# wenet-e2e/wenet

Hardware: AMD Instinct MI355X
Metric: audio-seconds/sec (RTF^-1), 12L Conformer fbank80, ctc_prefix_beam_search (higher is better)
Workload: dtype f32 (feed-forward and subsampling-conv2 GEMMs: fp32 operands as three exact bf16 planes, six plane products on the bf16 matrix cores, f32 accumulate -- error <= the v_mfma_f32 kernel's, tests/test_gpu_x6.py; everything else v_mfma_f32)

## Files before the change

### include/wenet_amd.h

```cpp
#ifndef WENET_AMD_H_
#define WENET_AMD_H_

#include <stdint.h>

#ifdef __cplusplus
extern "C" {
#endif

typedef struct wn_model wn_model;

typedef struct {
  int32_t feat_dim;
  int32_t d_model;
  int32_t n_heads;
  int32_t ffn_dim;
  int32_t n_layers;
  int32_t cnn_kernel;
  int32_t causal;
  int32_t use_dynamic_chunk;
  int32_t static_chunk_size;
  int32_t vocab;
  int32_t has_cmvn;
  int32_t dec_heads;
  int32_t dec_ffn_dim;
// ... 179 lines not shown
                    const float* resid_dev, float* C_dev, int32_t M, int32_t N,
                    int32_t K, float alpha, int32_t act, void* stream);
int wn_op_gemm_skinny(const float* A_dev, const float* W_dev, const float* bias_dev,
                      const float* resid_dev, float* C_dev, int32_t M, int32_t N, int32_t K,
                      int32_t act, int32_t w_bf16, int32_t split_k, void* stream);
int wn_op_gemm_bf16_stored(const float* A_dev, const float* W_dev, const float* bias_dev,
                           const float* resid_dev, void* C_dev, int32_t M, int32_t N,
                           int32_t K, float alpha, int32_t act, int32_t c_bf16,
                           void* stream);
int wn_op_gemm_lowp(const void* A_dev, const void* W_dev, const void* a_scale_dev,
                    const void* w_scale_dev, const float* bias_dev,
                    const float* resid_dev, void* C_dev, void* c_scale_dev, int32_t M,
                    int32_t N, int32_t K, float alpha, int32_t act, int32_t c_mode,
                    int32_t dtype, void* stream);
int wn_op_mx_quantize(const float* x_dev, int32_t rows, int32_t K, void* q_dev,
                      void* scale_dev, void* stream);
int wn_op_ffn_fused(const float* X_dev, const float* W1_dev, const float* b1_dev,
                    const float* W2_dev, const float* b2_dev, float* x_inout_dev,
                    const float* ln_w_dev, const float* ln_b_dev, float* y_out_dev,
                    int32_t M, int32_t D, int32_t F, int32_t act, float alpha, float eps,
                    void* stream);
int wn_op_gemm_x6(const float* A_dev, const float* W_dev, const float* bias_dev,
                  const float* resid_dev, float* C_dev, int32_t M, int32_t N, int32_t K,
                  float alpha, int32_t act, int32_t bm, int32_t reps, void* stream);
int wn_op_ffn_x6(const float* X_dev, const float* W1_dev, const float* b1_dev,
                 const float* W2_dev, const float* b2_dev, float* x_inout_dev,
                 const float* ln_w_dev, const float* ln_b_dev, float* y_out_dev, int32_t M,
                 int32_t D, int32_t F, int32_t act, float alpha, float eps, int32_t reps,
                 void* stream);
int wn_op_gemm_x6r(const float* A_dev, const float* W_dev, const float* bias_dev,
                   float* x_inout_dev, const float* ln_w_dev, const float* ln_b_dev,
                   float* y_dev, float* C_dev, int32_t M, int32_t N, int32_t epi, float alpha,
                   float eps, int32_t reps, void* stream);

int wn_op_gemm_x6r512(const float* A, const float* W, const float* bias, float* x_inout,
                      const float* ln_w, const float* ln_b, float* y, const float* W2,
                      const float* bias2, float* C, int32_t M, int32_t N, int32_t epi, float alpha,
                      float eps, int32_t reps, void* stream);
int wn_op_log_add(const double* a_dev, const double* b_dev, double* out_dev,
                  int32_t n, void* stream);
int wn_op_layernorm(const float* x_dev, const float* w_dev, const float* b_dev,
                    float* y_dev, int32_t M, int32_t D, float eps, void* stream);

typedef struct wn_attention_op {
  const void* Q; const void* K; const void* V;
  int32_t ldq, ldk, ldv;
  int32_t q_rows, kv_rows;
  const float* P; int32_t ldp, p_rows;
  const int32_t* p_off;
  const float* bias_u; const float* bias_v;
  void* O; int32_t ldo;
  const int32_t* q_off; const int32_t* q_len;
  const int32_t* kv_off; const int32_t* kv_len;
  int32_t n_seq, n_heads;
  int32_t mask_mode, chunk_size, left_chunks;
  float scale;
  int32_t flags;
  int32_t precision;
  int32_t x6_galign;
} wn_attention_op;
#define WN_ATTN_FOLD 1
#define WN_ATTN_PREFOLD 2
#define WN_ATTN_QKV_BF16 4
#define WN_ATTN_O_BF16 8
int wn_op_attention(const wn_attention_op* op, int32_t* form_out, void* stream);
int wn_op_dwconv(const float* x, int32_t ldx, const float* wt, const float* bias,
// ... 59 lines not shown
```

### wenet_amd/_lib.py

```python
import ctypes
import os
from ctypes import (POINTER, Structure, c_char_p, c_double, c_float, c_int32,
                    c_int64, c_void_p)

_HERE = os.path.dirname(os.path.abspath(__file__))
LIB_PATH = os.path.join(_HERE, 'libwenet_amd.so')


class WnConfig(Structure):
    _fields_ = [(n, c_int32) for n in (
        'feat_dim', 'd_model', 'n_heads', 'ffn_dim', 'n_layers', 'cnn_kernel',
        'causal', 'use_dynamic_chunk', 'static_chunk_size', 'vocab',
        'has_cmvn', 'dec_heads', 'dec_ffn_dim', 'dec_layers', 'dec_r_layers',
        'bidirectional', 'sos', 'eos', 'max_pos')] + [('norm_eps', c_float)] + [
            (n, c_int32) for n in ('encoder_type', 'input_layer', 'activation',
                                   'key_bias', 'cnn_norm',
                                   'dec_activation', 'dec_key_bias', 'dec_src_key_bias',
                                   'dec_learned_pos', 'dec_max_pos')]


class WnTransducerConfig(Structure):
    _fields_ = [(n, c_int32) for n in ('pred_embed', 'pred_hidden', 'pred_layers', 'pred_out',
                                       'join_dim', 'blank')]


class WnTensor(Structure):
    _fields_ = [('name', c_char_p), ('data', POINTER(c_float)),
                ('numel', c_int64)]


class WnStreamResult(Structure):
    _fields_ = [('n_hyps', POINTER(c_int32)), ('hyp_lens', POINTER(c_int32)),
                ('hyp_tlens', POINTER(c_int32)), ('hyp_tokens', POINTER(c_int32)),
                ('hyp_times', POINTER(c_int32)), ('hyp_scores', POINTER(c_double)),
                ('hyp_viterbi', POINTER(c_double)), ('frames_decoded', POINTER(c_int32)),
                ('trailing_blank', POINTER(c_int32)), ('max_len', c_int32)]


class WnAttentionOp(Structure):
    _fields_ = [('Q', c_void_p), ('K', c_void_p), ('V', c_void_p),
                ('ldq', c_int32), ('ldk', c_int32), ('ldv', c_int32),
                ('q_rows', c_int32), ('kv_rows', c_int32),
                ('P', c_void_p), ('ldp', c_int32), ('p_rows', c_int32),
                ('p_off', POINTER(c_int32)), ('bias_u', c_void_p), ('bias_v', c_void_p),
                ('O', c_void_p), ('ldo', c_int32),
                ('q_off', POINTER(c_int32)), ('q_len', POINTER(c_int32)),
                ('kv_off', POINTER(c_int32)), ('kv_len', POINTER(c_int32)),
                ('n_seq', c_int32), ('n_heads', c_int32), ('mask_mode', c_int32),
                ('chunk_size', c_int32), ('left_chunks', c_int32), ('scale', c_float),
                ('flags', c_int32), ('precision', c_int32), ('x6_galign', c_int32)]


EXPORTS = [
    'wn_last_error', 'wn_version', 'wn_model_create', 'wn_model_destroy', 'wn_model_clone',
    'wn_model_set_precision', 'wn_model_get_precision', 'wn_batch_size', 'wn_model_set_encode_gate', 'wn_op_gemm_bf16',
    'wn_op_gemm_bf16_stored',
    'wn_attention_beam_search', 'wn_attention_beam_search_prompt', 'wn_attention_truncated',
    'wn_op_gemm_skinny', 'wn_encode_chunk_batch', 'wn_op_gemm_lowp', 'wn_op_mx_quantize', 'wn_op_ffn_fused', 'wn_op_gemm_x6', 'wn_op_ffn_x6', 'wn_op_gemm_x6r', 'wn_op_gemm_x6r512', 'wn_profile_kernel_name', 'wn_profile_ffn_split', 'wn_profile_ffn_clocks', 'wn_profile_gemm_clocks', 'wn_filter_blank_embedding',
    'wn_workspace_create', 'wn_resample_length', 'wn_resample', 'wn_fbank', 'wn_log_mel', 'wn_encode', 'wn_encode_chunk', 'wn_set_encoder_out',
    'wn_ctc_logprobs', 'wn_set_ctc_probs', 'wn_ctc_greedy_search', 'wn_ctc_force_align',
    'wn_set_context_graph', 'wn_ctc_prefix_beam_search', 'wn_attention_rescoring', 'wn_rescore', 'wn_rescore_prefetch', 'wn_decoder_forward', 'wn_decoder_next_topk', 'wn_op_gemm',
    'wn_op_layernorm', 'wn_op_log_add', 'wn_op_attention', 'wn_op_dwconv', 'wn_op_conv1',
    'wn_op_ctc_rows', 'wn_debug_set', 'wn_profile_enable',
    'wn_profile_collect', 'wn_tune_set', 'wn_model_tune_set', 'wn_tune_get',
    'wn_stream_create', 'wn_stream_destroy', 'wn_stream_set_endpoint', 'wn_stream_reset',
    'wn_stream_advance', 'wn_stream_advance_encoded',
    'wn_model_create_transducer', 'wn_transducer_greedy_search', 'wn_op_lstm_step',
    'wn_op_joint_argmax',
]

_lib = None


def lib():
    global _lib
    if _lib is not None:
        return _lib
    if not os.path.exists(LIB_PATH):
        raise RuntimeError(
            f'{LIB_PATH} is missing: build it with `python -m wenet_amd.build` '
            '(hipcc --offload-arch=gfx950). wenet_amd has no CPU fallback.')
    import torch
    L = ctypes.CDLL(LIB_PATH, mode=ctypes.RTLD_GLOBAL)
    i32, i64, f32, vp = c_int32, c_int64, c_float, c_void_p
    pi32, pf64 = POINTER(c_int32), POINTER(c_double)
    L.wn_last_error.restype = c_char_p
    L.wn_profile_kernel_name.restype = c_char_p
    L.wn_profile_kernel_name.argtypes = [vp]
    L.wn_profile_ffn_split.restype = c_int32
    L.wn_profile_ffn_split.argtypes = [vp]
    L.wn_profile_ffn_clocks.argtypes = [POINTER(ctypes.c_uint64)]
# ... 29 lines not shown
    L.wn_stream_create.argtypes = [vp, i32, i32, i32, i32, POINTER(vp), vp]
    L.wn_stream_destroy.argtypes = [vp]
    L.wn_stream_set_endpoint.argtypes = [vp, f32, f32]
    L.wn_stream_reset.argtypes = [vp, i32, pi32, vp]
    L.wn_stream_advance.argtypes = [vp, i32, pi32, vp, pi32, i32, i32, i32,
                                    POINTER(WnStreamResult), vp]
    L.wn_stream_advance_encoded.argtypes = [vp, i32, pi32, vp, pi32, i32, i32,
                                            POINTER(WnStreamResult), vp]
    L.wn_attention_rescoring.argtypes = [vp, i32, pi32, pi32, pi32, i32, f32,
                                         POINTER(f32), POINTER(f32), vp]
    L.wn_rescore.argtypes = [vp, i32, pi32, pi32, pi32, pf64, i32, c_double, c_double, pi32,
                             POINTER(f32), pf64, pf64, POINTER(f32), vp]
    L.wn_rescore_prefetch.argtypes = [vp, i32, vp]
    L.wn_decoder_forward.argtypes = [vp, i32, i32, i32, pi32, pi32, i32, vp, vp]
    L.wn_decoder_next_topk.argtypes = [vp, i32, pi32, pi32, pi32, i32, i32,
                                       POINTER(f32), pi32, vp]
    L.wn_attention_beam_search.argtypes = [vp, i32, i32, f32, pi32, pi32, vp]
    L.wn_attention_beam_search_prompt.argtypes = [vp, i32, i32, f32, pi32, i32, pi32, pi32, vp]
    L.wn_attention_truncated.argtypes = [vp]
    L.wn_op_gemm.argtypes = [vp, vp, vp, vp, vp, i32, i32, i32, f32, i32, vp]
    L.wn_op_gemm_skinny.argtypes = [vp, vp, vp, vp, vp, i32, i32, i32, i32, i32, i32, vp]
    L.wn_op_gemm_bf16.argtypes = L.wn_op_gemm.argtypes
    L.wn_op_gemm_bf16_stored.argtypes = [vp, vp, vp, vp, vp, i32, i32, i32, f32, i32, i32, vp]
    L.wn_op_gemm_lowp.argtypes = [vp, vp, vp, vp, vp, vp, vp, vp, i32, i32, i32, f32, i32, i32,
                                  i32, vp]
    L.wn_op_mx_quantize.argtypes = [vp, i32, i32, vp, vp, vp]
    L.wn_op_ffn_fused.argtypes = [vp, vp, vp, vp, vp, vp, vp, vp, vp, i32, i32, i32, i32, f32,
                                  f32, vp]
    L.wn_op_gemm_x6.argtypes = [vp, vp, vp, vp, vp, i32, i32, i32, f32, i32, i32, i32, vp]
    L.wn_op_ffn_x6.argtypes = [vp, vp, vp, vp, vp, vp, vp, vp, vp, i32, i32, i32, i32, f32,
                               f32, i32, vp]
    L.wn_filter_blank_embedding.argtypes = [vp, vp, pi32, pi32, vp]
    L.wn_op_gemm_x6r.argtypes = [vp, vp, vp, vp, vp, vp, vp, vp, i32, i32, i32, f32, f32, i32, vp]
    L.wn_op_gemm_x6r512.argtypes = [vp, vp, vp, vp, vp, vp, vp, vp, vp, vp, i32, i32, i32, f32, f32,
                                    i32, vp]
    L.wn_model_set_precision.argtypes = [vp, i32]
    L.wn_model_get_precision.argtypes = [vp]
    L.wn_batch_size.argtypes = [vp]
    L.wn_batch_size.restype = i32
    L.wn_model_set_encode_gate.argtypes = [vp, vp]
    L.wn_op_layernorm.argtypes = [vp, vp, vp, vp, i32, i32, f32, vp]
    L.wn_op_log_add.argtypes = [vp, vp, vp, i32, vp]
    L.wn_op_attention.argtypes = [POINTER(WnAttentionOp), pi32, vp]
    L.wn_op_dwconv.argtypes = [vp, i32, vp, vp, vp, vp, vp, i32, vp, i32, pi32, pi32, i32, i32,
                               i32, i32, i32, i32, f32, vp]
    L.wn_op_conv1.argtypes = [vp, vp, vp, vp, vp, vp, pi32, pi32, i32, i32, i32, i32, i32, i32,
                              vp]
    L.wn_op_ctc_rows.argtypes = [vp, i32, i32, i32, i32, i32, f32, vp, vp, vp, i32, vp]
    L.wn_debug_set.argtypes = [vp, c_char_p, i32]
    L.wn_tune_set.argtypes = [c_char_p, i32]
    L.wn_model_tune_set.argtypes = [vp, c_char_p, i32]
    L.wn_tune_get.argtypes = [vp, c_char_p, pi32]
    L.wn_profile_enable.argtypes = [vp, i32]
    L.wn_profile_collect.argtypes = [vp, pi32, pf64, pf64]
    L.wn_model_create_transducer.argtypes = [POINTER(WnConfig), POINTER(WnTransducerConfig),
                                             POINTER(WnTensor), i32, i32, POINTER(vp)]
    L.wn_transducer_greedy_search.argtypes = [vp, i32, pi32, pi32, i32, pi32, vp]
    L.wn_op_lstm_step.argtypes = [vp, POINTER(vp), i32, vp, vp, vp, vp, vp, vp, i32, i32, i32,
                                  i32, vp]
    L.wn_op_joint_argmax.argtypes = [vp, i32, vp, i32, pi32, pi32, vp, vp, i32, i32, i32, pi32,
                                     POINTER(f32), vp]
    for n in EXPORTS:
        if n not in ('wn_last_error', 'wn_version', 'wn_model_destroy',
                     'wn_resample_length', 'wn_profile_kernel_name',
                     'wn_profile_ffn_split'):
            getattr(L, n).restype = i32
# ... 29 lines not shown
```

### wenet_amd/csrc/cabi_ops.hip

```cpp
#include "model_state.h"
#include "x6.h"

namespace wn {
namespace {

__global__ __launch_bounds__(256) void conv1_image_unpack_kernel(
    const char* __restrict__ img, int tiles, const int* __restrict__ t1_off,
    const int* __restrict__ t1_len, int F1, int C, float* __restrict__ out) {
  const int b = blockIdx.y;
  const int n = t1_len[b] * F1 * (C / 8);
  const int ne = (F1 + 1) / 2;
  for (int i = blockIdx.x * 256 + threadIdx.x; i < n; i += gridDim.x * 256) {
    const int cg = i % (C / 8), px = i / (C / 8);
    const int fr = px / F1, pos = px - fr * F1;
    const int f1 = pos < ne ? 2 * pos : 2 * (pos - ne) + 1;
    const int row = (t1_off[b] + fr) * F1;
    const char* src = img + x3_piece(cg >> 1, tiles, row + pos, cg & 1);
    const bf16x8 p0 = *reinterpret_cast<const bf16x8*>(src);
    const bf16x8 p1 = *reinterpret_cast<const bf16x8*>(src + X3_REC);
    const bf16x8 p2 = *reinterpret_cast<const bf16x8*>(src + 2 * X3_REC);
    float* o = out + ((int64_t)row + f1) * C + cg * 8;
#pragma unroll
    for (int e = 0; e < 8; ++e) o[e] = ((float)p0[e] + (float)p1[e]) + (float)p2[e];
  }
// ... 210 lines not shown
      g1.A = X; g1.lda = D; g1.a_bytes = (int64_t)M * D * 4;
      g1.epi = 0; g1.C = hf.as<float>(); g1.ldc = F;
      g2.A = hf.as<float>(); g2.lda = F; g2.a_bytes = (int64_t)M * F * 4;
    } else {
      WN_TRY(x6_split(X, M, D, D, x3.as<char>(), s));
      g1.A3 = x3.as<char>(); g1.epi = 2; g1.C3 = h3.as<char>();
      g2.A3 = h3.as<char>();
    }
    WN_TRY(gemm_x6(g1, s));
    WN_TRY(gemm_x6(g2, s));
    if (r + 1 < reps) continue;
    WN_TRY(ffn_reduce_ln(x, part.as<float>(), S, b2, alpha, ln_w, ln_b, nullptr, nullptr, y,
                         M, D, eps, 0, s));
  }
  return 0;
}

int wn_op_gemm_x6r(const float* A, const float* W, const float* bias, float* x_inout,
                   const float* ln_w, const float* ln_b, float* y, float* C, int32_t M,
                   int32_t N, int32_t epi, float alpha, float eps, int32_t reps, void* stream) {
  WN_CHECK(A && W && M > 0 && gemm_x6r_supported(M, N, 256, epi), "gemm_x6r: shape");
  hipStream_t s = (hipStream_t)stream;
  static thread_local DevBuf w3;
  WN_TRY(w3.ensure(x6_bytes(N, 256)));
  WN_TRY(x6_split(W, N, 256, 256, w3.as<char>(), s));
  X6RArgs a;
  a.A = A; a.lda = 256; a.W3 = w3.as<char>(); a.bias = bias; a.M = M; a.N = N; a.epi = epi;
  a.C = C; a.ldc = N; a.resid = x_inout; a.ldr = N; a.alpha = alpha; a.x_out = x_inout;
  a.ldx = N; a.ln_w = ln_w; a.ln_b = ln_b; a.eps = eps; a.y = y; a.ldy = N;
  for (int r = 0; r < (reps > 0 ? reps : 1); ++r) WN_TRY(gemm_x6r(a, s));
  return 0;
}

int wn_op_gemm_x6r512(const float* A, const float* W, const float* bias, float* x_inout,
                      const float* ln_w, const float* ln_b, float* y, const float* W2,
                      const float* bias2, float* C, int32_t M, int32_t N, int32_t epi, float alpha,
                      float eps, int32_t reps, void* stream) {
  WN_CHECK(A && W && M > 0 && gemm_x6r512_supported(M, N, epi), "gemm_x6r512: shape");
  WN_CHECK(epi != 3 || (W2 && C), "gemm_x6r512: the chained epilogue needs W2 and C");
  hipStream_t s = (hipStream_t)stream;
  static thread_local DevBuf w3, w3b;
  WN_TRY(w3.ensure(x6_bytes(N, 512)));
  WN_TRY(x6_split(W, N, 512, 512, w3.as<char>(), s));
  X6RArgs a;
  a.A = A; a.lda = 512; a.K = 512; a.W3 = w3.as<char>(); a.bias = bias; a.M = M; a.N = N;
  a.epi = epi; a.C = C; a.ldc = epi == 3 ? 512 : N; a.resid = x_inout; a.ldr = N; a.alpha = alpha;
  a.x_out = x_inout; a.ldx = N; a.ln_w = ln_w; a.ln_b = ln_b; a.eps = eps; a.y = y; a.ldy = N;
  if (epi == 3) {
    WN_TRY(w3b.ensure(x6_bytes(1024, 512)));
    WN_TRY(x6_split(W2, 1024, 512, 512, w3b.as<char>(), s));
    a.W3b = w3b.as<char>(); a.bias2 = bias2;
  }
  for (int r = 0; r < (reps > 0 ? reps : 1); ++r) WN_TRY(gemm_x6r(a, s));
  return 0;
}

int wn_op_log_add(const double* a_dev, const double* b_dev, double* out_dev,
                  int32_t n, void* stream) {
  return log_add_pairs(a_dev, b_dev, out_dev, n, (hipStream_t)stream);
}

int wn_op_layernorm(const float* x, const float* w, const float* b, float* y,
                    int32_t M, int32_t D, float eps, void* stream) {
  return layernorm(x, D, w, b, y, D, M, D, eps, (hipStream_t)stream);
}

// ... 197 lines not shown
```

### wenet_amd/csrc/gemm_x6r.hip

```cpp
#include "common.h"
#include "kernels.h"
#include "rowregs.h"
#include "attn_x6_img.h"
#include "x6.h"

namespace wn {

namespace {

#define WAVE_LDS_ORDER() asm volatile("s_waitcnt lgkmcnt(0)" ::: "memory")

constexpr int RK = 256;
constexpr int RKB = RK / 16;

__device__ unsigned long long g_x6r_clk[8][8];
template <int NT, int EPI, int PF, int PRO = 0>
__global__ __launch_bounds__(256, 1) void x6r_kernel(X6RArgs p) {
  const bool stamp = blockIdx.x == gridDim.x / 2 && threadIdx.x == 0;
  unsigned long long k0 = __builtin_readcyclecounter(), k1 = 0, k2 = 0, k3 = 0, k4 = 0, kp = 0;
  const unsigned long long rt0 = __builtin_amdgcn_s_memrealtime();
  __shared__ float red[2][4][32];
  constexpr int PATCH = 4 * 32 * (NT * 128 + 16) > 32 * 1040 ? 4 * 32 * (NT * 128 + 16) : 32 * 1040;
  __shared__ __attribute__((aligned(16))) char patch[PATCH];
  __shared__ __attribute__((aligned(16))) char ximg[RKB * 3 * 1024];
  const int tid = threadIdx.x, lane = tid & 63;
  const int wave = __builtin_amdgcn_readfirstlane(tid >> 6);
  __builtin_assume(wave >= 0 && wave < 4);
  const int hi = lane >> 5, li = lane & 31;
  const int m0 = blockIdx.x * 32;
  const int row = m0 + li;
  const int rowc = min(row, p.M - 1);

  {
    f32x4 rowv[8];
    if constexpr (PRO == 1) {
      const int c = lane * 4;
      const f32x4 b2 = *reinterpret_cast<const f32x4*>(p.pro_b2 + c);
      f32x4 acc8[8], xo8[8];
      int r8[8];
#pragma unroll
      for (int j = 0; j < 8; ++j) {
        r8[j] = min(m0 + wave * 8 + j, p.M - 1);
        acc8[j] = b2;
        xo8[j] = *reinterpret_cast<const f32x4*>(p.pro_x + (int64_t)r8[j] * RK + c);
      }
      int sl = 0;
      for (; sl + 4 <= p.pro_S; sl += 4) {
        f32x4 v[4][8];
#pragma unroll
        for (int u = 0; u < 4; ++u)
#pragma unroll
          for (int j = 0; j < 8; ++j)
            v[u][j] = *reinterpret_cast<const f32x4*>(
                p.pro_P + ((int64_t)(sl + u) * p.M + r8[j]) * RK + c);
#pragma unroll
        for (int u = 0; u < 4; ++u)
#pragma unroll
          for (int j = 0; j < 8; ++j) acc8[j] += v[u][j];
      }
      for (; sl < p.pro_S; ++sl) {
        f32x4 v[8];
#pragma unroll
        for (int j = 0; j < 8; ++j)
          v[j] = *reinterpret_cast<const f32x4*>(p.pro_P + ((int64_t)sl * p.M + r8[j]) * RK + c);
#pragma unroll
        for (int j = 0; j < 8; ++j) acc8[j] += v[j];
      }
// ... 139 lines not shown
        RowRegs<4> ww, bb;
        ww.load(a.ln_w, lane);
        bb.load(a.ln_b, lane);
#pragma unroll
        for (int r = 0; r < R; ++r) {
          const float var = sq[r] * (1.0f / RK);
          const float rstd = 1.0f / sqrtf(var + a.eps);
#pragma unroll
          for (int e = 0; e < 4; ++e)
            acc[r].v[e] = (acc[r].v[e] - sm[r]) * rstd * ww.v[e] + bb.v[e];
        }
      } else {
        RowRegs<4> sc, sh;
        sc.load(a.ln_w, lane);
        sh.load(a.ln_b, lane);
#pragma unroll
        for (int r = 0; r < R; ++r)
#pragma unroll
          for (int e = 0; e < 4; ++e) acc[r].v[e] = fmaf(acc[r].v[e], sc.v[e], sh.v[e]);
      }
#pragma unroll
      for (int r = 0; r < R; ++r)
#pragma unroll
        for (int e = 0; e < 4; ++e) rowv[r][e] = on[r] ? silu_f(acc[r].v[e]) : 0.f;
    } else {
#pragma unroll
      for (int j = 0; j < 8; ++j) {
        const int r = min(m0 + wave * 8 + j, p.M - 1);
        rowv[j] = *reinterpret_cast<const f32x4*>(p.A + (int64_t)r * p.lda + lane * 4);
      }
    }
    asm volatile("" : "+v"(rowv[0]), "+v"(rowv[7]));
    kp = __builtin_readcyclecounter();
#pragma unroll
    for (int j = 0; j < 8; ++j)
      *reinterpret_cast<f32x4*>(patch + (wave * 8 + j) * 1040 + lane * 16) = rowv[j];
  }
  const int Tn = (p.N + 31) >> 5;
  const char* wb = reinterpret_cast<const char*>(p.W3) + ((int64_t)wave * NT * 3) * X3_REC +
                   lane * 16;
  const int64_t kstride = (int64_t)Tn * X3_TILE;
  bf16x8 wf[PF + 1][NT][3];
  auto load_w = [&](int ks) {
    const char* q = wb + ks * kstride;
#pragma unroll
    for (int t = 0; t < NT; ++t)
#pragma unroll
      for (int pl = 0; pl < 3; ++pl)
        wf[ks % (PF + 1)][t][pl] = *reinterpret_cast<const bf16x8*>(q + (t * 3 + pl) * X3_REC);
  };
  constexpr bool RELOAD = PF == 1;
  auto load_rec = [&](int ks, int t, int pl) {
    wf[ks % (PF + 1)][t][pl] =
        *reinterpret_cast<const bf16x8*>(wb + ks * kstride + (t * 3 + pl) * X3_REC);
  };
  __builtin_amdgcn_sched_barrier(0);
#pragma unroll
  for (int s = 0; s < (RELOAD ? 2 : PF); ++s) load_w(s);
  __syncthreads();
  k1 = __builtin_readcyclecounter();
  auto split_quarter = [&]() {
#pragma unroll
    for (int j = 0; j < RKB / 4; ++j) {
      const int ks = wave * (RKB / 4) + j;
      const f32x4 a4 = *reinterpret_cast<const f32x4*>(patch + li * 1040 + ks * 64 + hi * 32);
      const f32x4 b4 = *reinterpret_cast<const f32x4*>(patch + li * 1040 + ks * 64 + hi * 32 + 16);
      bf16x8 x3[3];
#pragma unroll
      for (int e = 0; e < 4; ++e) {
        const Split3 sa = split3(a4[e]), sb = split3(b4[e]);
        x3[0][e] = sa.h0; x3[1][e] = sa.h1; x3[2][e] = sa.h2;
        x3[0][4 + e] = sb.h0; x3[1][4 + e] = sb.h1; x3[2][4 + e] = sb.h2;
      }
#pragma unroll
      for (int pl = 0; pl < 3; ++pl)
        *reinterpret_cast<bf16x8*>(ximg + (ks * 3 + pl) * 1024 + lane * 16) = x3[pl];
    }
  };
  bf16x8 xf[2][3];
  auto load_x = [&](int ks) {
#pragma unroll
    for (int pl = 0; pl < 3; ++pl)
      xf[ks & 1][pl] = *reinterpret_cast<const bf16x8*>(ximg + (ks * 3 + pl) * 1024 + lane * 16);
  };
  split_quarter();
  __syncthreads();
  load_x(0);

  f32x16 acc[NT];
#pragma unroll
  for (int t = 0; t < NT; ++t)
#pragma unroll
    for (int r = 0; r < 16; ++r) acc[t][r] = 0.f;
  const int ecol = wave * NT * 32 + 4 * hi;
  f32x4 ebias[NT][4], elw[(EPI == 1 || EPI == 3) ? NT : 1][4], elb[(EPI == 1 || EPI == 3) ? NT : 1][4];
#pragma unroll
  for (int t = 0; t < NT; ++t)
#pragma unroll
    for (int g = 0; g < 4; ++g) {
      const int c = min(ecol + t * 32 + 8 * g, p.N - 4);
      ebias[t][g] = f32x4{0.f, 0.f, 0.f, 0.f};
      if (p.bias) ebias[t][g] = *reinterpret_cast<const f32x4*>(p.bias + c);
      if constexpr (EPI == 1 || EPI == 3) {
        elw[t][g] = *reinterpret_cast<const f32x4*>(p.ln_w + c);
        elb[t][g] = *reinterpret_cast<const f32x4*>(p.ln_b + c);
      }
    }
  k2 = __builtin_readcyclecounter();

  constexpr int PW[6] = {2, 0, 1, 1, 0, 0}, PX[6] = {0, 2, 1, 0, 1, 0};
#pragma unroll
  for (int ks = 0; ks < RKB; ++ks) {
    if (!RELOAD && ks + PF < RKB) load_w(ks + PF);
    if (ks + 1 < RKB) load_x(ks + 1);
#pragma unroll
    for (int q = 0; q < 6; ++q) {
#pragma unroll
      for (int t = 0; t < NT; ++t)
        acc[t] = __builtin_amdgcn_mfma_f32_32x32x16_bf16(wf[ks % (PF + 1)][t][PW[q]],
                                                         xf[ks & 1][PX[q]], acc[t], 0, 0, 0);
      if (RELOAD && ks + 2 < RKB && (q == 0 || q == 3 || q == 5)) {
        __builtin_amdgcn_sched_barrier(0);
#pragma unroll
        for (int t = 0; t < NT; ++t) load_rec(ks + 2, t, q == 0 ? 2 : q == 3 ? 1 : 0);
      }
    }
    __builtin_amdgcn_sched_barrier(0);
  }

  asm volatile("" : "+v"(acc[0]), "+v"(acc[NT - 1]));
  k3 = __builtin_readcyclecounter();
  const int col0 = wave * NT * 32;
  constexpr int SEG = NT * 128;
  constexpr int PST = SEG + 16;
  constexpr int LPR = SEG / 16;
  constexpr int NIT = 32 * LPR / 64;
  __syncthreads();
  char* wp = patch + wave * (32 * PST);
  auto put = [&](const f32x4 (&v)[NT][4]) {
#pragma unroll
    for (int t = 0; t < NT; ++t)
#pragma unroll
      for (int g = 0; g < 4; ++g)
        *reinterpret_cast<f32x4*>(wp + li * PST + (t * 32 + 8 * g + 4 * hi) * 4) = v[t][g];
  };
  auto get = [&](f32x4 (&v)[NT][4]) {
#pragma unroll
    for (int t = 0; t < NT; ++t)
#pragma unroll
      for (int g = 0; g < 4; ++g)
        v[t][g] = *reinterpret_cast<const f32x4*>(wp + li * PST + (t * 32 + 8 * g + 4 * hi) * 4);
  };
  auto store_rows = [&](float* base, int ld) {
#pragma unroll
    for (int it = 0; it < NIT; ++it) {
      const int q = it * 64 + lane, r = q / LPR, pc = q - r * LPR;
      const f32x4 v = *reinterpret_cast<const f32x4*>(wp + r * PST + pc * 16);
      if (m0 + r < p.M && col0 + pc * 4 < p.N)
        *reinterpret_cast<f32x4*>(base + (int64_t)(m0 + r) * ld + col0 + pc * 4) = v;
    }
  };
  if constexpr (EPI == 0) {
    f32x4 v[NT][4];
#pragma unroll
    for (int t = 0; t < NT; ++t)
#pragma unroll
      for (int g = 0; g < 4; ++g) {
        v[t][g] = f32x4{acc[t][4 * g], acc[t][4 * g + 1], acc[t][4 * g + 2], acc[t][4 * g + 3]} +
                  ebias[t][g];
      }
    put(v);
// ... 167 lines not shown
      for (int g = 0; g < 4; ++g)
#pragma unroll
        for (int e = 0; e < 4; ++e) {
          const float d = v[t][g][e] - mean;
          s2 += d * d;
        }
    s2 += __shfl_xor(s2, 32, 64);
    if (hi == 0) red[1][wave][li] = s2;
    __syncthreads();
    const float var =
        ((red[1][0][li] + red[1][1][li]) + (red[1][2][li] + red[1][3][li])) / (float)p.N;
    const float rstd = 1.0f / sqrtf(var + p.eps);
#pragma unroll
    for (int t = 0; t < NT; ++t)
#pragma unroll
      for (int g = 0; g < 4; ++g) {
        const f32x4 w = elw[t][g], b = elb[t][g];
#pragma unroll
        for (int e = 0; e < 4; ++e) v[t][g][e] = (v[t][g][e] - mean) * rstd * w[e] + b[e];
      }
    if (p.y != nullptr) {
      put(v);
      store_rows(p.y, p.ldy);
    }
    if constexpr (EPI == 1) {
      if (p.y3 != nullptr) {
        const int tiles_m = (p.M + 31) >> 5;
#pragma unroll
        for (int t = 0; t < NT; ++t)
          x3_store_tile(v[t], p.y3, (col0 + t * 32) >> 4, tiles_m, blockIdx.x, hi, li);
      }
    }
    if constexpr (EPI == 3) {
      __syncthreads();
#pragma unroll
      for (int t = 0; t < NT; ++t)
#pragma unroll
        for (int g = 0; g < 4; ++g)
          *reinterpret_cast<f32x4*>(patch + li * 1040 + (col0 + t * 32 + 8 * g + 4 * hi) * 4) =
              v[t][g];
      constexpr int NT2 = 4, PF2 = 2;
      const char* wb2 = reinterpret_cast<const char*>(p.W3b) +
                        ((int64_t)wave * NT2 * 3) * X3_REC + lane * 16;
      const int64_t kstride2 = (int64_t)16 * X3_TILE;
      bf16x8 wf2[PF2 + 1][NT2][3];
      auto load_w2 = [&](int ks) {
        const char* q = wb2 + ks * kstride2;
#pragma unroll
        for (int t = 0; t < NT2; ++t)
#pragma unroll
          for (int pl = 0; pl < 3; ++pl)
            wf2[ks % (PF2 + 1)][t][pl] =
                *reinterpret_cast<const bf16x8*>(q + (t * 3 + pl) * X3_REC);
      };
#pragma unroll
      for (int s2i = 0; s2i < PF2; ++s2i) load_w2(s2i);
      __syncthreads();
      split_quarter();
      __syncthreads();
      load_x(0);
      f32x16 acc2[NT2];
#pragma unroll
      for (int t = 0; t < NT2; ++t)
#pragma unroll
        for (int r = 0; r < 16; ++r) acc2[t][r] = 0.f;
      f32x4 ebias2[NT2][4];
#pragma unroll
      for (int t = 0; t < NT2; ++t)
#pragma unroll
        for (int g = 0; g < 4; ++g) {
          ebias2[t][g] = f32x4{0.f, 0.f, 0.f, 0.f};
          if (p.bias2)
            ebias2[t][g] = *reinterpret_cast<const f32x4*>(p.bias2 + wave * NT2 * 32 + t * 32 +
                                                           8 * g + 4 * hi);
        }
#pragma unroll
      for (int ks = 0; ks < RKB; ++ks) {
        if (ks + PF2 < RKB) load_w2(ks + PF2);
        if (ks + 1 < RKB) load_x(ks + 1);
#pragma unroll
        for (int q = 0; q < 6; ++q)
#pragma unroll
          for (int t = 0; t < NT2; ++t)
            acc2[t] = __builtin_amdgcn_mfma_f32_32x32x16_bf16(wf2[ks % (PF2 + 1)][t][PW[q]],
                                                              xf[ks & 1][PX[q]], acc2[t], 0, 0, 0);
        __builtin_amdgcn_sched_barrier(0);
      }
      __syncthreads();
      const int c2 = wave * NT2 * 32;
      char* wp2 = patch + wave * (32 * 272);
#pragma unroll
      for (int u = 0; u < 2; ++u)
#pragma unroll
        for (int g = 0; g < 4; ++g) {
          const int c = c2 + 2 * u * 32 + 8 * g + 4 * hi;
          f32x4 a = f32x4{acc2[2 * u][4 * g], acc2[2 * u][4 * g + 1], acc2[2 * u][4 * g + 2],
                          acc2[2 * u][4 * g + 3]};
          f32x4 gt = f32x4{acc2[2 * u + 1][4 * g], acc2[2 * u + 1][4 * g + 1],
                           acc2[2 * u + 1][4 * g + 2], acc2[2 * u + 1][4 * g + 3]};
          a += ebias2[2 * u][g];
          gt += ebias2[2 * u + 1][g];
          f32x4 o;
#pragma unroll
          for (int e = 0; e < 4; ++e) o[e] = a[e] * wn_rcp(1.0f + wn_exp(-gt[e]));
          *reinterpret_cast<f32x4*>(wp2 + li * 272 + (u * 32 + 8 * g + 4 * hi) * 4) = o;
        }
#pragma unroll
      for (int it = 0; it < 8; ++it) {
        const int q = it * 64 + lane, r = q >> 4, pc = q & 15;
        const f32x4 o = *reinterpret_cast<const f32x4*>(wp2 + r * 272 + pc * 16);
        if (m0 + r < p.M)
          *reinterpret_cast<f32x4*>(p.C + (int64_t)(m0 + r) * p.ldc + c2 / 2 + pc * 4) = o;
      }
    }
  }
  asm volatile("s_waitcnt vmcnt(0)" ::: "memory");
  k4 = __builtin_readcyclecounter();
  if (stamp) {
    unsigned long long* o = g_x6r_clk[(EPI == 4 ? 0 : EPI) + (PRO != 0 ? 4 : 0)];
    o[0] = k0; o[1] = k1; o[2] = k2; o[3] = k3; o[4] = k4; o[5] = kp;
    o[6] = rt0; o[7] = __builtin_amdgcn_s_memrealtime();
  }
}

template <int NT, int EPI, int PF, int PRO = 0>
int launch_x6r(const X6RArgs& a, hipStream_t s) {
  hipLaunchKernelGGL((x6r_kernel<NT, EPI, PF, PRO>), dim3(cdiv(a.M, 32)), dim3(256), 0, s, a);
  WN_HIP(hipGetLastError());
  return 0;
}

}

int gemm_x6r_clocks(unsigned long long* out) {
  WN_HIP(hipDeviceSynchronize());
  WN_HIP(hipMemcpyFromSymbol(out, HIP_SYMBOL(g_x6r_clk), sizeof(g_x6r_clk)));
  return 0;
}

bool gemm_x6r_supported(int M, int N, int K, int epi) {
  if (K == 512) return gemm_x6r512_supported(M, N, epi);
  if (K != RK || M <= 0) return false;
  if (epi == 1 || epi == 3) return N == 256;
  if (epi == 2) return N == 512;
  if (epi == 4) return N == 768;
  return N == 256 || N == 512 || N == 768;
}

int gemm_x6r(const X6RArgs& a, hipStream_t s) {
  if (a.K == 512) return gemm_x6r512(a, s);
  WN_CHECK(a.K == RK, "gemm_x6r: K must be 256 or 512");
  if (a.pro_P) {
    WN_CHECK((a.epi == 0 || a.epi == 4) && a.N == 768 && a.W3 && a.M > 0 && a.pro_S >= 1 &&
                 a.pro_b2 && a.pro_x && a.ln_w && a.ln_b && a.C && a.ldc % 4 == 0,
             "gemm_x6r: prologue fold arguments");
    if (a.epi == 4) {
      WN_CHECK(a.at_img && a.at_P && a.at_ldp % 4 == 0 && a.at_u && a.at_v && a.at_row_utt &&
                   a.at_off && a.bias, "gemm_x6r: key-tile image arguments (epi 4)");
      return launch_x6r<6, 4, 1, 1>(a, s);
    }
    return launch_x6r<6, 0, 1, 1>(a, s);
  }
  WN_CHECK((a.A || a.dw_on) && a.W3 && a.lda % 4 == 0 && a.epi != 4 &&
               gemm_x6r_supported(a.M, a.N, RK, a.epi), "gemm_x6r: shape");
  if (a.dw_on) {
    WN_CHECK(a.epi == 1 && a.N == 256 && a.W3 && a.M > 0 && a.dw.D == 256 && a.dw.M == a.M &&
                 a.dw.x && a.dw.ldx % 4 == 0 && a.dw.wt && a.dw.bias && a.dw.cpad && a.dw.ln_w &&
                 a.dw.ln_b && a.dw.row_utt && a.dw.off && a.dw.len && a.dw.K >= 1 &&
                 a.resid && a.x_out && a.ln_w && a.ln_b && (a.y || a.y3) && a.ldr % 4 == 0 &&
// ... 25 lines not shown
```

### wenet_amd/csrc/kernels.h

```cpp
#pragma once
#include "common.h"

namespace wn {

int layernorm(const float* x, int ldx, const float* w, const float* b, float* y,
              int ldy, int M, int D, float eps, hipStream_t s, bool y_bf16 = false);

int layernorm_mx(const float* x, int ldx, const float* w, const float* b, void* q,
                 unsigned* scale, int pitch, int M, int D, float eps, hipStream_t s);

int layernorm2(const float* x, const float* w1, const float* b1, const float* w2,
               const float* b2, float* y1, float* y2, int M, int D, float eps,
               hipStream_t s, bool y2_bf16 = false);

struct Conv1Args {
  const float* feats;
  const float* mean;
  const float* istd;
  const float* w;
  const float* bias;
  float* out;
  char* out3 = nullptr;
  int tiles = 0;
  const int* t1_off;
// ... 140 lines not shown
  const float* W;
  const float* bias;
  const float* resid; int ldr;
  float alpha;
  float* x_out; int ldx;
  const float* ln_w; const float* ln_b; float eps;
  float* y; int ldy;
  int M, N, K;
};
struct X6RArgs {
  const float* A = nullptr; int lda = 0;
  int K = 256;
  const void* W3 = nullptr;
  const float* bias = nullptr;
  int M = 0, N = 0;
  int epi = 0;
  float* C = nullptr; int ldc = 0;
  const float* resid = nullptr; int ldr = 0; float alpha = 1.0f;
  float* x_out = nullptr; int ldx = 0;
  const float* ln_w = nullptr; const float* ln_b = nullptr; float eps = 1e-5f;
  float* y = nullptr; int ldy = 0;
  void* y3 = nullptr;
  const void* W3b = nullptr; const float* bias2 = nullptr;
  const float* pro_P = nullptr; int pro_S = 0; const float* pro_b2 = nullptr;
  float pro_alpha = 0.f; float* pro_x = nullptr;
  int dw_on = 0;
  DwConvArgs dw;
  void* at_img = nullptr;
  const float* at_P = nullptr; int at_ldp = 0;
  const float* at_u = nullptr; const float* at_v = nullptr;
  const int* at_row_utt = nullptr; const int* at_off = nullptr; const int* at_p_off = nullptr;
};
int gemm_x6r_clocks(unsigned long long* out);
bool gemm_x6r_supported(int M, int N, int K, int epi);
int gemm_x6r(const X6RArgs& a, hipStream_t s);
bool gemm_x6r512_supported(int M, int N, int epi);
int gemm_x6r512(const X6RArgs& a, hipStream_t s);
bool gemm_rowln_supported(int M, int N, int K);
int gemm_rowln(const RowLnArgs& a, hipStream_t s);

struct CtcRowArgs {
  const float* logits; int ld;
  int M, V, k;
  int blank; float blank_penalty;
  float* topk_val;
  int* topk_idx;
  float* logp;
  int ld_out;
};
int ctc_logsoftmax_topk(const CtcRowArgs& a, hipStream_t s);

int nonblank_map(const int* top1, int stride, const int* off, const int* len, int B, int* map,
                 int* n_keep, hipStream_t s);
int nonblank_gather(const float* src, const int* map, const int* off, const int* n_keep,
                    const int* noff, const int* nlen, const int* row_utt_new, float* dst, int D,
                    int rows_new, hipStream_t s);
int ctc_greedy_collapse(const int* top1, int top1_stride, const int* off,
                        const int* len, int B, int blank, int* out_tokens,
                        int out_stride, int* out_lens, hipStream_t s);

struct CtxGraph {
  const int* fail = nullptr;
  const double* node_score = nullptr;
  const double* output_score = nullptr;
  const double* token_score = nullptr;
  const unsigned long long* keys = nullptr;
// ... 182 lines not shown
```

Measured before the change: 72900.

## Shrink x6r NT=2 shared memory to allow two blocks per CU

For the NT=2 instantiations of the x6r GEMM kernel, the fp32 row patch is halved (stride 528 instead of 1040) and the bf16 plane split runs in two passes, with each half of the row staged in turn. The reduction scratch is aliased into the patch, epilogue staging moves into the ximg buffer, and bias2 is staged through shared memory instead of held in registers. Launch bounds are raised to 2 blocks per CU so two workgroups can co-reside and hide latency. The extra passes add barriers. The change also adds an extended C entry point and a resource query for registers, LDS and occupancy.

Result: no change. 72640 (median of 2 runs) (-0.4%).

```diff
diff --git a/include/wenet_amd.h b/include/wenet_amd.h
--- a/include/wenet_amd.h
+++ b/include/wenet_amd.h
@@ -235,6 +235,21 @@
                    float* x_inout_dev, const float* ln_w_dev, const float* ln_b_dev,
                    float* y_dev, float* C_dev, int32_t M, int32_t N, int32_t epi, float alpha,
                    float eps, int32_t reps, void* stream);
+typedef struct {
+  const float* A; const float* W; const float* bias; float* x_inout;
+  const float* ln_w; const float* ln_b; float* y; float* C;
+  int32_t M, N, epi; float alpha, eps;
+  const float* W2; const float* bias2;
+  int32_t dw_on;
+  const float* dw_x; int32_t dw_ldx;
+  const float* dw_wt; const float* dw_bias; const float* dw_cpad;
+  const float* dw_ln_w; const float* dw_ln_b;
+  int32_t dw_norm_mode;
+  const int32_t* dw_off; const int32_t* dw_len;
+  int32_t dw_B, dw_K, dw_causal, dw_t_max; float dw_eps;
+} wn_x6r_op;
+int wn_op_gemm_x6r_ex(const wn_x6r_op* op, void* stream);
+int wn_op_x6r_resources(int32_t epi, int32_t dw_on, int32_t out[4]);
 
 int wn_op_gemm_x6r512(const float* A, const float* W, const float* bias, float* x_inout,
                       const float* ln_w, const float* ln_b, float* y, const float* W2,
diff --git a/wenet_amd/_lib.py b/wenet_amd/_lib.py
--- a/wenet_amd/_lib.py
+++ b/wenet_amd/_lib.py
@@ -51,12 +51,26 @@
                 ('flags', c_int32), ('precision', c_int32), ('x6_galign', c_int32)]
 
 
+class WnX6rOp(Structure):
+    _fields_ = [('A', c_void_p), ('W', c_void_p), ('bias', c_void_p), ('x_inout', c_void_p),
+                ('ln_w', c_void_p), ('ln_b', c_void_p), ('y', c_void_p), ('C', c_void_p),
+                ('M', c_int32), ('N', c_int32), ('epi', c_int32),
+                ('alpha', c_float), ('eps', c_float),
+                ('W2', c_void_p), ('bias2', c_void_p), ('dw_on', c_int32),
+                ('dw_x', c_void_p), ('dw_ldx', c_int32),
+                ('dw_wt', c_void_p), ('dw_bias', c_void_p), ('dw_cpad', c_void_p),
+                ('dw_ln_w', c_void_p), ('dw_ln_b', c_void_p), ('dw_norm_mode', c_int32),
+                ('dw_off', POINTER(c_int32)), ('dw_len', POINTER(c_int32)),
+                ('dw_B', c_int32), ('dw_K', c_int32), ('dw_causal', c_int32),
+                ('dw_t_max', c_int32), ('dw_eps', c_float)]
+
+
 EXPORTS = [
     'wn_last_error', 'wn_version', 'wn_model_create', 'wn_model_destroy', 'wn_model_clone',
     'wn_model_set_precision', 'wn_model_get_precision', 'wn_batch_size', 'wn_model_set_encode_gate', 'wn_op_gemm_bf16',
     'wn_op_gemm_bf16_stored',
     'wn_attention_beam_search', 'wn_attention_beam_search_prompt', 'wn_attention_truncated',
-    'wn_op_gemm_skinny', 'wn_encode_chunk_batch', 'wn_op_gemm_lowp', 'wn_op_mx_quantize', 'wn_op_ffn_fused', 'wn_op_gemm_x6', 'wn_op_ffn_x6', 'wn_op_gemm_x6r', 'wn_op_gemm_x6r512', 'wn_profile_kernel_name', 'wn_profile_ffn_split', 'wn_profile_ffn_clocks', 'wn_profile_gemm_clocks', 'wn_filter_blank_embedding',
+    'wn_op_gemm_skinny', 'wn_encode_chunk_batch', 'wn_op_gemm_lowp', 'wn_op_mx_quantize', 'wn_op_ffn_fused', 'wn_op_gemm_x6', 'wn_op_ffn_x6', 'wn_op_gemm_x6r', 'wn_op_gemm_x6r_ex', 'wn_op_x6r_resources', 'wn_op_gemm_x6r512', 'wn_profile_kernel_name', 'wn_profile_ffn_split', 'wn_profile_ffn_clocks', 'wn_profile_gemm_clocks', 'wn_filter_blank_embedding',
     'wn_workspace_create', 'wn_resample_length', 'wn_resample', 'wn_fbank', 'wn_log_mel', 'wn_encode', 'wn_encode_chunk', 'wn_set_encoder_out',
     'wn_ctc_logprobs', 'wn_set_ctc_probs', 'wn_ctc_greedy_search', 'wn_ctc_force_align',
     'wn_set_context_graph', 'wn_ctc_prefix_beam_search', 'wn_attention_rescoring', 'wn_rescore', 'wn_rescore_prefetch', 'wn_decoder_forward', 'wn_decoder_next_topk', 'wn_op_gemm',
@@ -152,6 +166,8 @@
                                f32, i32, vp]
     L.wn_filter_blank_embedding.argtypes = [vp, vp, pi32, pi32, vp]
     L.wn_op_gemm_x6r.argtypes = [vp, vp, vp, vp, vp, vp, vp, vp, i32, i32, i32, f32, f32, i32, vp]
+    L.wn_op_gemm_x6r_ex.argtypes = [POINTER(WnX6rOp), vp]
+    L.wn_op_x6r_resources.argtypes = [i32, i32, pi32]
     L.wn_op_gemm_x6r512.argtypes = [vp, vp, vp, vp, vp, vp, vp, vp, vp, vp, i32, i32, i32, f32, f32,
                                     i32, vp]
     L.wn_model_set_precision.argtypes = [vp, i32]
diff --git a/wenet_amd/csrc/cabi_ops.hip b/wenet_amd/csrc/cabi_ops.hip
--- a/wenet_amd/csrc/cabi_ops.hip
+++ b/wenet_amd/csrc/cabi_ops.hip
@@ -266,6 +266,61 @@
   return 0;
 }
 
+int wn_op_gemm_x6r_ex(const wn_x6r_op* op, void* stream) {
+  WN_CHECK(op, "gemm_x6r: null argument");
+  const wn_x6r_op& o = *op;
+  WN_CHECK((o.A || o.dw_on) && o.W && o.M > 0 && gemm_x6r_supported(o.M, o.N, 256, o.epi),
+           "gemm_x6r: shape");
+  WN_CHECK(o.epi != 3 || (o.W2 && o.C), "gemm_x6r: the chained epilogue needs W2 and C");
+  hipStream_t s = (hipStream_t)stream;
+  static thread_local DevBuf w3, w3b, desc;
+  WN_TRY(w3.ensure(x6_bytes(o.N, 256)));
+  WN_TRY(x6_split(o.W, o.N, 256, 256, w3.as<char>(), s));
+  X6RArgs a;
+  a.A = o.A; a.lda = 256; a.W3 = w3.as<char>(); a.bias = o.bias; a.M = o.M; a.N = o.N;
+  a.epi = o.epi; a.C = o.C; a.ldc = o.epi == 3 ? 256 : o.N; a.resid = o.x_inout; a.ldr = o.N;
+  a.alpha = o.alpha; a.x_out = o.x_inout; a.ldx = o.N; a.ln_w = o.ln_w; a.ln_b = o.ln_b;
+  a.eps = o.eps; a.y = o.y; a.ldy = o.N;
+  if (o.epi == 3) {
+    WN_TRY(w3b.ensure(x6_bytes(512, 256)));
+    WN_TRY(x6_split(o.W2, 512, 256, 256, w3b.as<char>(), s));
+    a.W3b = w3b.as<char>(); a.bias2 = o.bias2;
+  }
+  if (o.dw_on) {
+    const int B = o.dw_B, M = o.M;
+    WN_CHECK(o.dw_x && o.dw_wt && o.dw_bias && o.dw_cpad && o.dw_ln_w && o.dw_ln_b && o.dw_off &&
+                 o.dw_len, "gemm_x6r: null depthwise-conv argument");
+    WN_CHECK(B > 0 && o.dw_K >= 1 && o.dw_K <= 255 && (o.dw_causal != 0 || o.dw_K % 2 == 1) &&
+                 o.dw_ldx % 4 == 0 && o.dw_ldx >= 256 &&
+                 (o.dw_norm_mode == 0 || o.dw_norm_mode == 1), "gemm_x6r: depthwise-conv shape");
+    WN_CHECK(packed_ok(o.dw_off, o.dw_len, B, M),
+             "gemm_x6r: rows outside the buffer, unordered or overlapping");
+    std::vector<int> h((size_t)2 * B + M, -1);
+    for (int b = 0; b < B; ++b) {
+      WN_CHECK(o.dw_len[b] <= o.dw_t_max, "gemm_x6r: t_max is smaller than a length");
+      h[b] = o.dw_off[b]; h[B + b] = o.dw_len[b];
+      for (int t = 0; t < o.dw_len[b]; ++t) h[2 * B + o.dw_off[b] + t] = b;
+    }
+    WN_TRY(upload_ints(desc, h, s));
+    DwConvArgs& d = a.dw;
+    d.x = o.dw_x; d.ldx = o.dw_ldx; d.wt = o.dw_wt; d.bias = o.dw_bias; d.cpad = o.dw_cpad;
+    d.ln_w = o.dw_ln_w; d.ln_b = o.dw_ln_b; d.norm_mode = o.dw_norm_mode; d.y = nullptr; d.ldy = 0;
+    d.off = desc.as<int>(); d.len = d.off + B; d.row_utt = d.off + 2 * B;
+    d.M = M; d.D = 256; d.K = o.dw_K; d.causal = o.dw_causal != 0; d.t_max = o.dw_t_max;
+    d.eps = o.dw_eps;
+    a.dw_on = 1;
+  }
+  return gemm_x6r(a, s);
+}
+
+int wn_op_x6r_resources(int32_t epi, int32_t dw_on, int32_t out[4]) {
+  WN_CHECK(out, "x6r_resources: null argument");
+  int r[4];
+  WN_TRY(gemm_x6r_resources(epi, dw_on != 0, r));
+  for (int i = 0; i < 4; ++i) out[i] = r[i];
+  return 0;
+}
+
 int wn_op_gemm_x6r512(const float* A, const float* W, const float* bias, float* x_inout,
                       const float* ln_w, const float* ln_b, float* y, const float* W2,
                       const float* bias2, float* C, int32_t M, int32_t N, int32_t epi, float alpha,
diff --git a/wenet_amd/csrc/gemm_x6r.hip b/wenet_amd/csrc/gemm_x6r.hip
--- a/wenet_amd/csrc/gemm_x6r.hip
+++ b/wenet_amd/csrc/gemm_x6r.hip
@@ -15,13 +15,17 @@
 
 __device__ unsigned long long g_x6r_clk[8][8];
 template <int NT, int EPI, int PF, int PRO = 0>
-__global__ __launch_bounds__(256, 1) void x6r_kernel(X6RArgs p) {
+__global__ __launch_bounds__(256, NT == 2 ? 2 : 1) void x6r_kernel(X6RArgs p) {
   const bool stamp = blockIdx.x == gridDim.x / 2 && threadIdx.x == 0;
   unsigned long long k0 = __builtin_readcyclecounter(), k1 = 0, k2 = 0, k3 = 0, k4 = 0, kp = 0;
   const unsigned long long rt0 = __builtin_amdgcn_s_memrealtime();
-  __shared__ float red[2][4][32];
-  constexpr int PATCH = 4 * 32 * (NT * 128 + 16) > 32 * 1040 ? 4 * 32 * (NT * 128 + 16) : 32 * 1040;
+  constexpr bool PAIR = NT == 2;
+  constexpr int AST = PAIR ? 528 : 1040;
+  constexpr int PATCH = PAIR ? 32 * AST
+                             : 4 * 32 * (NT * 128 + 16) > 32 * 1040 ? 4 * 32 * (NT * 128 + 16) : 32 * 1040;
   __shared__ __attribute__((aligned(16))) char patch[PATCH];
+  static_assert((EPI != 1 && EPI != 3) || PAIR, "the LayerNorm forms: NT = 2");
+  float (*red)[4][32] = reinterpret_cast<float (*)[4][32]>(patch);
   __shared__ __attribute__((aligned(16))) char ximg[RKB * 3 * 1024];
   const int tid = threadIdx.x, lane = tid & 63;
   const int wave = __builtin_amdgcn_readfirstlane(tid >> 6);
@@ -31,8 +35,8 @@
   const int row = m0 + li;
   const int rowc = min(row, p.M - 1);
 
+  f32x4 rowv[8];
   {
-    f32x4 rowv[8];
     if constexpr (PRO == 1) {
       const int c = lane * 4;
       const f32x4 b2 = *reinterpret_cast<const f32x4*>(p.pro_b2 + c);
@@ -238,9 +242,11 @@
     }
     asm volatile("" : "+v"(rowv[0]), "+v"(rowv[7]));
     kp = __builtin_readcyclecounter();
-#pragma unroll
-    for (int j = 0; j < 8; ++j)
-      *reinterpret_cast<f32x4*>(patch + (wave * 8 + j) * 1040 + lane * 16) = rowv[j];
+    if (!PAIR || hi == 0) {
+#pragma unroll
+      for (int j = 0; j < 8; ++j)
+        *reinterpret_cast<f32x4*>(patch + (wave * 8 + j) * AST + lane * 16) = rowv[j];
+    }
   }
   const int Tn = (p.N + 31) >> 5;
   const char* wb = reinterpret_cast<const char*>(p.W3) + ((int64_t)wave * NT * 3) * X3_REC +
@@ -265,12 +271,14 @@
   for (int s = 0; s < (RELOAD ? 2 : PF); ++s) load_w(s);
   __syncthreads();
   k1 = __builtin_readcyclecounter();
-  auto split_quarter = [&]() {
-#pragma unroll
-    for (int j = 0; j < RKB / 4; ++j) {
-      const int ks = wave * (RKB / 4) + j;
-      const f32x4 a4 = *reinterpret_cast<const f32x4*>(patch + li * 1040 + ks * 64 + hi * 32);
-      const f32x4 b4 = *reinterpret_cast<const f32x4*>(patch + li * 1040 + ks * 64 + hi * 32 + 16);
+  constexpr int NSPL = PAIR ? 2 : 4;
+  auto split_blocks = [&](int ks0) {
+#pragma unroll
+    for (int j = 0; j < NSPL; ++j) {
+      const int ks = ks0 + wave * NSPL + j;
+      const int ac = (PAIR ? ks & 7 : ks) * 64 + hi * 32;
+      const f32x4 a4 = *reinterpret_cast<const f32x4*>(patch + li * AST + ac);
+      const f32x4 b4 = *reinterpret_cast<const f32x4*>(patch + li * AST + ac + 16);
       bf16x8 x3[3];
 #pragma unroll
       for (int e = 0; e < 4; ++e) {
@@ -289,8 +297,18 @@
     for (int pl = 0; pl < 3; ++pl)
       xf[ks & 1][pl] = *reinterpret_cast<const bf16x8*>(ximg + (ks * 3 + pl) * 1024 + lane * 16);
   };
-  split_quarter();
+  split_blocks(0);
   __syncthreads();
+  if constexpr (PAIR) {
+    if (hi == 1) {
+#pragma unroll
+      for (int j = 0; j < 8; ++j)
+        *reinterpret_cast<f32x4*>(patch + (wave * 8 + j) * AST + li * 16) = rowv[j];
+    }
+    __syncthreads();
+    split_blocks(8);
+    __syncthreads();
+  }
   load_x(0);
 
   f32x16 acc[NT];
@@ -342,7 +360,7 @@
   constexpr int LPR = SEG / 16;
   constexpr int NIT = 32 * LPR / 64;
   __syncthreads();
-  char* wp = patch + wave * (32 * PST);
+  char* wp = (PAIR ? ximg : patch) + wave * (32 * PST);
   auto put = [&](const f32x4 (&v)[NT][4]) {
 #pragma unroll
     for (int t = 0; t < NT; ++t)
@@ -576,13 +594,17 @@
       }
     }
     if constexpr (EPI == 3) {
+      static_assert(EPI != 3 || PAIR, "chained form: NT = 2");
+      auto put_y = [&]() {
+#pragma unroll
+        for (int t = 0; t < NT; ++t)
+#pragma unroll
+          for (int g = 0; g < 4; ++g)
+            *reinterpret_cast<f32x4*>(patch + li * AST +
+                                      ((col0 & 127) + t * 32 + 8 * g + 4 * hi) * 4) = v[t][g];
+      };
       __syncthreads();
-#pragma unroll
-      for (int t = 0; t < NT; ++t)
-#pragma unroll
-        for (int g = 0; g < 4; ++g)
-          *reinterpret_cast<f32x4*>(patch + li * 1040 + (col0 + t * 32 + 8 * g + 4 * hi) * 4) =
-              v[t][g];
+      if (wave < 2) put_y();
       constexpr int NT2 = 4, PF2 = 2;
       const char* wb2 = reinterpret_cast<const char*>(p.W3b) +
                         ((int64_t)wave * NT2 * 3) * X3_REC + lane * 16;
@@ -599,25 +621,22 @@
       };
 #pragma unroll
       for (int s2i = 0; s2i < PF2; ++s2i) load_w2(s2i);
+      f32x4 b2v = f32x4{0.f, 0.f, 0.f, 0.f};
+      if (p.bias2 && tid < 128) b2v = *reinterpret_cast<const f32x4*>(p.bias2 + tid * 4);
       __syncthreads();
-      split_quarter();
+      split_blocks(0);
       __syncthreads();
+      if (wave >= 2) put_y();
+      __syncthreads();
+      split_blocks(8);
+      __syncthreads();
+      if (tid < 128) *reinterpret_cast<f32x4*>(patch + tid * 16) = b2v;
       load_x(0);
       f32x16 acc2[NT2];
 #pragma unroll
       for (int t = 0; t < NT2; ++t)
 #pragma unroll
         for (int r = 0; r < 16; ++r) acc2[t][r] = 0.f;
-      f32x4 ebias2[NT2][4];
-#pragma unroll
-      for (int t = 0; t < NT2; ++t)
-#pragma unroll
-        for (int g = 0; g < 4; ++g) {
-          ebias2[t][g] = f32x4{0.f, 0.f, 0.f, 0.f};
-          if (p.bias2)
-            ebias2[t][g] = *reinterpret_cast<const f32x4*>(p.bias2 + wave * NT2 * 32 + t * 32 +
-                                                           8 * g + 4 * hi);
-        }
 #pragma unroll
       for (int ks = 0; ks < RKB; ++ks) {
         if (ks + PF2 < RKB) load_w2(ks + PF2);
@@ -632,7 +651,14 @@
       }
       __syncthreads();
       const int c2 = wave * NT2 * 32;
-      char* wp2 = patch + wave * (32 * 272);
+      char* wp2 = ximg + wave * (32 * 272);
+      f32x4 ebias2[NT2][4];
+#pragma unroll
+      for (int t = 0; t < NT2; ++t)
+#pragma unroll
+        for (int g = 0; g < 4; ++g)
+          ebias2[t][g] =
+              *reinterpret_cast<const f32x4*>(patch + (c2 + t * 32 + 8 * g + 4 * hi) * 4);
 #pragma unroll
       for (int u = 0; u < 2; ++u)
 #pragma unroll
@@ -679,6 +705,29 @@
 int gemm_x6r_clocks(unsigned long long* out) {
   WN_HIP(hipDeviceSynchronize());
   WN_HIP(hipMemcpyFromSymbol(out, HIP_SYMBOL(g_x6r_clk), sizeof(g_x6r_clk)));
+  return 0;
+}
+
+int gemm_x6r_resources(int epi, bool dw_on, int out[4]) {
+  const void* f = nullptr;
+  if (dw_on) {
+    WN_CHECK(epi == 1, "gemm_x6r_resources: the depthwise-conv prologue comes with epi 1");
+    f = reinterpret_cast<const void*>(&x6r_kernel<2, 1, 3, 2>);
+  } else {
+    switch (epi) {
+      case 0: f = reinterpret_cast<const void*>(&x6r_kernel<2, 0, 3>); break;
+      case 1: f = reinterpret_cast<const void*>(&x6r_kernel<2, 1, 3>); break;
+      case 3: f = reinterpret_cast<const void*>(&x6r_kernel<2, 3, 3>); break;
+      case 4: f = reinterpret_cast<const void*>(&x6r_kernel<6, 4, 1, 1>); break;
+      default: WN_CHECK(false, "gemm_x6r_resources: epi must be 0, 1, 3 or 4");
+    }
+  }
+  hipFuncAttributes at;
+  WN_HIP(hipFuncGetAttributes(&at, f));
+  int blocks = 0;
+  WN_HIP(hipOccupancyMaxActiveBlocksPerMultiprocessor(&blocks, f, 256, 0));
+  out[0] = at.numRegs; out[1] = (int)at.sharedSizeBytes; out[2] = (int)at.localSizeBytes;
+  out[3] = blocks;
   return 0;
 }
 
diff --git a/wenet_amd/csrc/kernels.h b/wenet_amd/csrc/kernels.h
--- a/wenet_amd/csrc/kernels.h
+++ b/wenet_amd/csrc/kernels.h
@@ -196,6 +196,7 @@
   const int* at_row_utt = nullptr; const int* at_off = nullptr; const int* at_p_off = nullptr;
 };
 int gemm_x6r_clocks(unsigned long long* out);
+int gemm_x6r_resources(int epi, bool dw_on, int out[4]);
 bool gemm_x6r_supported(int M, int N, int K, int epi);
 int gemm_x6r(const X6RArgs& a, hipStream_t s);
 bool gemm_x6r512_supported(int M, int N, int epi);
```
